# ariel415el/SoundEventDetection-Pytorch

Hardware: AMD Instinct MI355X
Metric: SED train clips/sec (60s,64-mel,9-layer CNN) (higher is better)
Workload: dtype bf16; 1 GPU; Cnn_AvgPooling main widths [32, 64, 128, 128], 60 s / 32 kHz / 64-mel clips (T=6001 frames, NFFT 1024, hop 320), batch 32/GPU, train step = waveform->log-mel->fwd->BCE->bwd->Adam-amsgrad; frontend_constants=bench, graph_replay=False, global_batch=32, frames=6001, parallelism=dp1, frontend_in_step=True, frontend_overlapped=False, frontend_overlap_mode=0, sync_bn=False, rccl_group=False, collectives_executed=False

## Files before the change

### soundeventdetection-pytorch_amd/csrc/sed_c1.hip

```cpp
#include "conv_common.h"

constexpr int C1_TR = 8;

template <typename T>
__global__ __launch_bounds__(256) void conv_c1_fwd_kernel(const float* __restrict__ x, const float* __restrict__ mean,
                                                          const float* __restrict__ stdv, const float* __restrict__ w,
                                                          T* __restrict__ z, float* __restrict__ partial, int B,
                                                          int H, int W, int Cout, int Coutp, int G, int PPB) {
    extern __shared__ __attribute__((aligned(16))) char smem[];
    float* wsm = reinterpret_cast<float*>(smem);
    float* xrow = wsm + 9 * Coutp;
    float* red = xrow + (C1_TR + 2) * (W + 2);
    const int tid = threadIdx.x;
    for (int i = tid; i < 9 * Coutp; i += blockDim.x) {
        const int tap = i / Coutp, c = i % Coutp;
        wsm[i] = c < Cout ? w[c * 9 + tap] : 0.f;
    }
    __syncthreads();
    const int cg = tid % G, pl = tid / G;
    float wr[9][8];
#pragma unroll
    for (int t = 0; t < 9; ++t)
#pragma unroll
        for (int e = 0; e < 8; ++e) wr[t][e] = wsm[t * Coutp + cg * 8 + e];
    float S[8], Q[8];
#pragma unroll
    for (int e = 0; e < 8; ++e) { S[e] = 0.f; Q[e] = 0.f; }
    const int WP2 = W + 2;
    const int bands = (H + C1_TR - 1) / C1_TR;
    for (int band = blockIdx.x; band < B * bands; band += gridDim.x) {
        const int b = band / bands, h0 = (band - b * bands) * C1_TR;
        __syncthreads();
        for (int i = tid; i < (C1_TR + 2) * WP2; i += blockDim.x) {
            const int rr = i / WP2, cc = i - rr * WP2;
            const int hy = h0 + rr - 1, wx = cc - 1;
            float v = 0.f;
            if (hy >= 0 && hy < H && wx >= 0 && wx < W) {
                v = x[((size_t)b * H + hy) * W + wx];
                if (mean) v = (v - mean[wx]) / stdv[wx];
            }
            xrow[i] = v;
        }
        __syncthreads();
        if (pl < PPB) {
            for (int wq = pl; wq < W; wq += PPB) {
                float x0[3], x1[3], x2[3];
#pragma unroll
                for (int j = 0; j < 3; ++j) { x0[j] = xrow[wq + j]; x1[j] = xrow[WP2 + wq + j]; }
#pragma unroll
                for (int r = 0; r < C1_TR; ++r) {
#pragma unroll
                    for (int j = 0; j < 3; ++j) x2[j] = xrow[(r + 2) * WP2 + wq + j];
                    if (h0 + r < H) {
                        float a[8];
#pragma unroll
                        for (int e = 0; e < 8; ++e) a[e] = 0.f;
#pragma unroll
                        for (int j = 0; j < 3; ++j) {
#pragma unroll
                            for (int e = 0; e < 8; ++e) a[e] = fmaf(x0[j], wr[j][e], a[e]);
                        }
#pragma unroll
                        for (int j = 0; j < 3; ++j) {
#pragma unroll
                            for (int e = 0; e < 8; ++e) a[e] = fmaf(x1[j], wr[3 + j][e], a[e]);
                        }
#pragma unroll
                        for (int j = 0; j < 3; ++j) {
#pragma unroll
                            for (int e = 0; e < 8; ++e) a[e] = fmaf(x2[j], wr[6 + j][e], a[e]);
                        }
#pragma unroll
                        for (int e = 0; e < 8; ++e) { S[e] += a[e]; Q[e] = fmaf(a[e], a[e], Q[e]); }
                        store8<T>(z + (((size_t)b * H + h0 + r) * W + wq) * Coutp + cg * 8, a);
                    }
#pragma unroll
                    for (int j = 0; j < 3; ++j) { x0[j] = x1[j]; x1[j] = x2[j]; }
                }
            }
        }
    }
    if (partial) {
        __syncthreads();
        if (pl < PPB) {
#pragma unroll
            for (int e = 0; e < 8; ++e) {
                red[(pl * 2 + 0) * Coutp + cg * 8 + e] = S[e];
                red[(pl * 2 + 1) * Coutp + cg * 8 + e] = Q[e];
            }
        }
        __syncthreads();
        for (int i = tid; i < 2 * Coutp; i += blockDim.x) {
            float t = 0.f;
            for (int q = 0; q < PPB; ++q) t += red[q * 2 * Coutp + i];
            partial[(size_t)blockIdx.x * 2 * Coutp + i] = t;
        }
    }
}

template <typename T, bool FUSED, int NPF>
__global__ __launch_bounds__(256) void conv_c1_wgrad_kernel(const float* __restrict__ x, const float* __restrict__ mean,
                                                            const float* __restrict__ stdv, const T* __restrict__ dz,
                                                            const T* __restrict__ zsrc, const float* __restrict__ ca,
                                                            const float* __restrict__ cb, const float* __restrict__ cc,
                                                            float* __restrict__ partial, int B, int H, int W,
                                                            int Coutp, int G, int PPB) {
    extern __shared__ __attribute__((aligned(16))) char smem[];
    float* xrow = reinterpret_cast<float*>(smem);
    float* red = xrow + (C1_TR + 2) * (W + 2);
    const int tid = threadIdx.x;
    const int cg = tid % G, pl = tid / G;
    const int WP2 = W + 2;
    float acc[9][8];
#pragma unroll
    for (int t = 0; t < 9; ++t)
#pragma unroll
        for (int e = 0; e < 8; ++e) acc[t][e] = 0.f;
    float a8[8], b8[8], c8[8];
    if (FUSED) {
#pragma unroll
        for (int e = 0; e < 8; ++e) { a8[e] = ca[cg * 8 + e]; b8[e] = cb[cg * 8 + e]; c8[e] = cc[cg * 8 + e]; }
    }
    const int bands = (H + C1_TR - 1) / C1_TR;
    const int nstage = (C1_TR + 2) * WP2;
    float pf[NPF];
    auto fetch = [&](int band) {
        const int b = band / bands, h0 = (band - b * bands) * C1_TR;
#pragma unroll
        for (int u = 0; u < NPF; ++u) {
            const int i = tid + u * 256;
            const int rr = i / WP2, cc2 = i - rr * WP2;
            const int hy = h0 + rr - 1, wx = cc2 - 1;
            float v = 0.f;
            if (i < nstage && band < B * bands && hy >= 0 && hy < H && wx >= 0 && wx < W) {
                v = x[((size_t)b * H + hy) * W + wx];
                if (mean) v = (v - mean[wx]) / stdv[wx];
            }
            pf[u] = v;
        }
    };
    fetch(blockIdx.x);
    for (int band = blockIdx.x; band < B * bands; band += gridDim.x) {
        const int b = band / bands, h0 = (band - b * bands) * C1_TR;
        (void)b;
        __syncthreads();
#pragma unroll
        for (int u = 0; u < NPF; ++u)
            if (tid + u * 256 < nstage) xrow[tid + u * 256] = pf[u];
        __syncthreads();
        fetch(band + gridDim.x);
        if (pl < PPB) {
            for (int wq = pl; wq < W; wq += PPB) {
                float x0[3], x1[3], x2[3];
#pragma unroll
                for (int j = 0; j < 3; ++j) { x0[j] = xrow[wq + j]; x1[j] = xrow[WP2 + wq + j]; }
                float d[C1_TR][8], zz[FUSED ? C1_TR : 1][8];
#pragma unroll
                for (int r = 0; r < C1_TR; ++r) {
                    const int h = (h0 + r < H) ? h0 + r : H - 1;
                    const size_t off = (((size_t)b * H + h) * W + wq) * Coutp + cg * 8;
                    load8<T>(dz + off, d[r]);
                    if (FUSED) load8<T>(zsrc + off, zz[FUSED ? r : 0]);
                }
#pragma unroll
                for (int r = 0; r < C1_TR; ++r) {
#pragma unroll
                    for (int j = 0; j < 3; ++j) x2[j] = xrow[(r + 2) * WP2 + wq + j];
                    if (h0 + r < H) {
                        if (FUSED) {
#pragma unroll
                            for (int e = 0; e < 8; ++e) d[r][e] = fmaf(a8[e], d[r][e], fmaf(b8[e], zz[FUSED ? r : 0][e], c8[e]));
                        }
#pragma unroll
                        for (int j = 0; j < 3; ++j) {
#pragma unroll
                            for (int e = 0; e < 8; ++e) {
                                acc[j][e] = fmaf(x0[j], d[r][e], acc[j][e]);
                                acc[3 + j][e] = fmaf(x1[j], d[r][e], acc[3 + j][e]);
                                acc[6 + j][e] = fmaf(x2[j], d[r][e], acc[6 + j][e]);
                            }
                        }
                    }
#pragma unroll
                    for (int j = 0; j < 3; ++j) { x0[j] = x1[j]; x1[j] = x2[j]; }
                }
            }
        }
    }
#pragma unroll
    for (int t = 0; t < 9; ++t) {
        __syncthreads();
        if (pl < PPB) {
#pragma unroll
            for (int e = 0; e < 8; ++e) red[pl * Coutp + cg * 8 + e] = acc[t][e];
        }
        __syncthreads();
        for (int i = tid; i < Coutp; i += blockDim.x) {
            float sacc = 0.f;
            for (int q = 0; q < PPB; ++q) sacc += red[q * Coutp + i];
            partial[((size_t)blockIdx.x * 9 + t) * Coutp + i] = sacc;
        }
    }
}

template <int SIT>
__global__ __launch_bounds__(256) void conv_c1_gram_kernel(const float* __restrict__ x, const float* __restrict__ mean,
                                                           const float* __restrict__ stdv, float* __restrict__ partial,
                                                           int B, int H, int W) {
    extern __shared__ __attribute__((aligned(16))) char smem[];
    float* xrow = reinterpret_cast<float*>(smem);
    float* red = xrow + (C1_TR + 2) * (W + 2);
    const int tid = threadIdx.x, lane = tid & 63, wave = tid >> 6;
    const int WP2 = W + 2;
    float acc[54];
#pragma unroll
    for (int i = 0; i < 54; ++i) acc[i] = 0.f;
    const int bands = (H + C1_TR - 1) / C1_TR;
    int srow[SIT], scol[SIT];
    float smu[SIT], sinv[SIT];
#pragma unroll
    for (int u = 0; u < SIT; ++u) {
        const int i = tid + u * 256;
        const int rr = i / WP2, cc2 = i - rr * WP2;
        const bool ok = i < (C1_TR + 2) * WP2 && cc2 >= 1 && cc2 <= W;
        srow[u] = i < (C1_TR + 2) * WP2 ? rr - 1 : (1 << 28);
        scol[u] = ok ? cc2 - 1 : -1;
        smu[u] = (ok && mean) ? mean[cc2 - 1] : 0.f;
        sinv[u] = (ok && mean) ? 1.0f / stdv[cc2 - 1] : 1.f;
    }
    const int npix = C1_TR * W;
    float nraw[SIT];
    unsigned nvalid = 0;
    auto fetch = [&](int band) {
        nvalid = 0;
        if (band >= B * bands) return;
        const int b = band / bands, h0 = (band - b * bands) * C1_TR;
#pragma unroll
        for (int u = 0; u < SIT; ++u) {
            const int hy = h0 + srow[u];
            const bool ok = hy >= 0 && hy < H && scol[u] >= 0;
            nraw[u] = ok ? x[((size_t)b * H + hy) * W + scol[u]] : 0.f;
            nvalid |= ok ? (1u << u) : 0u;
        }
    };
    fetch(blockIdx.x);
    for (int band = blockIdx.x; band < B * bands; band += gridDim.x) {
        const int b = band / bands, h0 = (band - b * bands) * C1_TR;
        (void)b;
        __syncthreads();
#pragma unroll
        for (int u = 0; u < SIT; ++u) {
            const int i = tid + u * 256;
            if (i >= (C1_TR + 2) * WP2) break;
            xrow[i] = ((nvalid >> u) & 1u) ? (nraw[u] - smu[u]) * sinv[u] : 0.f;
        }
        fetch(band + gridDim.x);
        __syncthreads();
        for (int pix = tid; pix < npix; pix += blockDim.x) {
            const int r = pix / W, wq = pix - r * W;
            if (h0 + r >= H) continue;
            float xp[9];
#pragma unroll
            for (int t = 0; t < 9; ++t) xp[t] = xrow[(r + t / 3) * WP2 + wq + t % 3];
#pragma unroll
            for (int j = 0; j < 9; ++j)
#pragma unroll
                for (int k = j; k < 9; ++k) {
                    constexpr int dummy = 0; (void)dummy;
                    const int o = j * 9 - j * (j - 1) / 2 + (k - j);
                    acc[o] = fmaf(xp[j], xp[k], acc[o]);
                }
#pragma unroll
            for (int k = 0; k < 9; ++k) acc[45 + k] += xp[k];
        }
    }
    __syncthreads();
#pragma unroll
    for (int i = 0; i < 54; ++i) {
        const float t = wave_sum(acc[i]);
        if (lane == 0) red[wave * 54 + i] = t;
    }
    __syncthreads();
    if (tid < 54) partial[(size_t)blockIdx.x * 54 + tid] = red[tid] + red[54 + tid] + red[108 + tid] + red[162 + tid];
}

__global__ __launch_bounds__(1024) void bn_train_finalize_c1_kernel(const float* __restrict__ gram, int nparts, double count,
                                                                    const float* __restrict__ w, const float* __restrict__ gamma,
                                                                    const float* __restrict__ beta, float* __restrict__ rmean,
                                                                    float* __restrict__ rvar, float momentum, float eps,
                                                                    float* __restrict__ scale, float* __restrict__ shift,
                                                                    float* __restrict__ mean_o, float* __restrict__ invstd_o, int C,
                                                                    int Cp, double* __restrict__ gsum_out = nullptr) {
    __shared__ double G[54];
    __shared__ double Gp[16][64];
    const int tid = threadIdx.x;
    {
        const int v = tid & 63, g = tid >> 6;
        double s = 0.0;
        if (v < 54) {
            int i = g;
            for (; i + 16 * 7 < nparts; i += 16 * 8) {
                float t[8];
#pragma unroll
                for (int u = 0; u < 8; ++u) t[u] = gram[(size_t)(i + 16 * u) * 54 + v];
#pragma unroll
                for (int u = 0; u < 8; ++u) s += (double)t[u];
            }
            for (; i < nparts; i += 16) s += (double)gram[(size_t)i * 54 + v];
        }
        Gp[g][v] = s;
    }
    __syncthreads();
    if (tid < 54) {
        double s = 0.0;
        for (int g = 0; g < 16; ++g) s += Gp[g][tid];
        G[tid] = s;
        if (gsum_out != nullptr) gsum_out[tid] = s;
    }
    __syncthreads();
    for (int c = tid; c < Cp; c += blockDim.x) {
        if (c >= C) { scale[c] = 0.f; shift[c] = 0.f; mean_o[c] = 0.f; invstd_o[c] = 0.f; continue; }
        double s1 = 0.0, s2 = 0.0;
        for (int j = 0; j < 9; ++j) {
            s1 += (double)w[c * 9 + j] * G[45 + j];
            for (int k2 = 0; k2 < 9; ++k2) {
                const int a = j < k2 ? j : k2, b2 = j < k2 ? k2 : j;
                s2 += (double)w[c * 9 + j] * (double)w[c * 9 + k2] * G[a * 9 - a * (a - 1) / 2 + (b2 - a)];
            }
        }
        const double mean = s1 / count;
        double var = s2 / count - mean * mean;
        if (var < 0.0) var = 0.0;
        const float invstd = (float)(1.0 / sqrt(var + (double)eps));
        const float sc = gamma[c] * invstd;
        scale[c] = sc;
        shift[c] = beta[c] - (float)mean * sc;
        mean_o[c] = (float)mean;
        invstd_o[c] = invstd;
        if (rmean) {
            const double unbiased = count > 1.0 ? var * (count / (count - 1.0)) : var;
            rmean[c] = (1.f - momentum) * rmean[c] + momentum * (float)mean;
            rvar[c] = (1.f - momentum) * rvar[c] + momentum * (float)unbiased;
        }
    }
}

__global__ __launch_bounds__(256) void bn_bwd_finalize_c1_kernel(const float* __restrict__ partial, int nparts, double count,
                                                                 const float* __restrict__ A, const float* __restrict__ w,
                                                                 const float* __restrict__ gamma, const float* __restrict__ mean,
                                                                 const float* __restrict__ invstd, float* __restrict__ dgamma,
                                                                 float* __restrict__ dbeta, float* __restrict__ ca,
                                                                 float* __restrict__ cb, float* __restrict__ cc, int C, int Cp) {
    __shared__ double sm[256];
    const int c = blockIdx.x, tid = threadIdx.x;
    double s = 0.0;
    for (int i = tid; i < nparts; i += 256) s += (double)partial[((size_t)i * 2 + 0) * Cp + c];
    sm[tid] = s;
    __syncthreads();
    for (int o = 128; o > 0; o >>= 1) {
        if (tid < o) sm[tid] += sm[tid + o];
        __syncthreads();
    }
    if (tid == 0) {
        if (c >= C) { ca[c] = 0.f; cb[c] = 0.f; cc[c] = 0.f; return; }
        const double sg = sm[0];
        double sgz = 0.0;
        for (int k2 = 0; k2 < 9; ++k2) sgz += (double)w[c * 9 + k2] * (double)A[k2 * Cp + c];
        const double g = gamma[c], is = invstd[c], mu = mean[c];
        const double q = is * (sgz - mu * sg);
        dbeta[c] = (float)sg;
        dgamma[c] = (float)q;
        const double mg = sg / count, mgx = q / count;
        ca[c] = (float)(g * is);
        cb[c] = (float)(-g * is * is * mgx);
        cc[c] = (float)(-g * is * (mg - mu * is * mgx));
    }
}

__global__ __launch_bounds__(1024) void conv_c1_wgrad_combine_kernel(const float* __restrict__ A, const float* __restrict__ gram,
                                                                    int nparts, const float* __restrict__ w,
                                                                    const float* __restrict__ ca, const float* __restrict__ cb,
                                                                    const float* __restrict__ cc, float* __restrict__ dw,
                                                                    int Cout, int Coutp, float* __restrict__ dw_torch = nullptr) {
    __shared__ double G[54];
    __shared__ double Gp[16][64];
    const int tid = threadIdx.x;
    {
        const int v = tid & 63, g = tid >> 6;
        double s = 0.0;
        if (v < 54) {
            int i = g;
            for (; i + 16 * 7 < nparts; i += 16 * 8) {
                float t[8];
#pragma unroll
                for (int u = 0; u < 8; ++u) t[u] = gram[(size_t)(i + 16 * u) * 54 + v];
#pragma unroll
                for (int u = 0; u < 8; ++u) s += (double)t[u];
            }
            for (; i < nparts; i += 16) s += (double)gram[(size_t)i * 54 + v];
        }
        Gp[g][v] = s;
    }
    __syncthreads();
    if (tid < 54) {
        double s = 0.0;
        for (int g = 0; g < 16; ++g) s += Gp[g][tid];
        G[tid] = s;
    }
    __syncthreads();
    for (int idx = tid; idx < 9 * Coutp; idx += blockDim.x) {
        const int k = idx / Coutp, c = idx - k * Coutp;
        float out = 0.f;
        if (c < Cout) {
            double wg = 0.0;
            for (int j = 0; j < 9; ++j) {
                const int a = j < k ? j : k, b2 = j < k ? k : j;
                wg += (double)w[c * 9 + j] * G[a * 9 - a * (a - 1) / 2 + (b2 - a)];
            }
            out = (float)((double)ca[c] * (double)A[idx] + (double)cb[c] * wg + (double)cc[c] * G[45 + k]);
        }
        dw[idx] = out;
        if (dw_torch != nullptr && c < Cout) dw_torch[c * 9 + k] = out;
    }
}

__global__ __launch_bounds__(1024) void c1_bwd_tail_kernel(const float* __restrict__ a_part, int a_nparts, const double* __restrict__ gsum,
                                                           double count, const float* __restrict__ w, const float* __restrict__ gamma,
                                                           const float* __restrict__ mean, const float* __restrict__ invstd,
                                                           float* __restrict__ dgamma, float* __restrict__ dbeta, float* __restrict__ ca,
                                                           float* __restrict__ cb, float* __restrict__ cc, float* __restrict__ a10_out,
                                                           float* __restrict__ dw, int Cout, float* __restrict__ dw_torch) {
    constexpr int Cp = 32, NV = 10 * Cp, NG = 3;
    __shared__ double As[NG][NV];
    __shared__ float a10[NV];
    __shared__ float coef[3][Cp];
    __shared__ double G[54];
    const int tid = threadIdx.x;
    if (tid < 54) G[tid] = gsum[tid];
    if (tid < NG * NV) {
        const int v = tid % NV, g = tid / NV;
        double s = 0.0;
        int i = g;
        for (; i + NG * 7 < a_nparts; i += NG * 8) {
            float t[8];
#pragma unroll
            for (int u = 0; u < 8; ++u) t[u] = a_part[(size_t)(i + NG * u) * NV + v];
#pragma unroll
            for (int u = 0; u < 8; ++u) s += (double)t[u];
        }
        for (; i < a_nparts; i += NG) s += (double)a_part[(size_t)i * NV + v];
        As[g][v] = s;
    }
    __syncthreads();
    if (tid < NV) {
        const float t = (float)(As[0][tid] + As[1][tid] + As[2][tid]);
        a10[tid] = t;
        a10_out[tid] = t;
    }
    __syncthreads();
    if (tid < Cp) {
        const int c = tid;
        float fa = 0.f, fb = 0.f, fc = 0.f;
        if (c < Cout) {
            const double sg = (double)a10[9 * Cp + c];
            double sgz = 0.0;
            for (int k2 = 0; k2 < 9; ++k2) sgz += (double)w[c * 9 + k2] * (double)a10[k2 * Cp + c];
            const double g = gamma[c], is = invstd[c], mu = mean[c];
            const double q = is * (sgz - mu * sg);
            dbeta[c] = (float)sg;
            dgamma[c] = (float)q;
            const double mg = sg / count, mgx = q / count;
            fa = (float)(g * is);
            fb = (float)(-g * is * is * mgx);
            fc = (float)(-g * is * (mg - mu * is * mgx));
        }
        ca[c] = fa; cb[c] = fb; cc[c] = fc;
        coef[0][c] = fa; coef[1][c] = fb; coef[2][c] = fc;
    }
    __syncthreads();
    for (int idx = tid; idx < 9 * Cp; idx += blockDim.x) {
        const int k = idx / Cp, c = idx - k * Cp;
        float out = 0.f;
        if (c < Cout) {
            double wg = 0.0;
            for (int j = 0; j < 9; ++j) {
                const int a = j < k ? j : k, b2 = j < k ? k : j;
                wg += (double)w[c * 9 + j] * G[a * 9 - a * (a - 1) / 2 + (b2 - a)];
            }
            out = (float)((double)coef[0][c] * (double)a10[idx] + (double)coef[1][c] * wg + (double)coef[2][c] * G[45 + k]);
        }
        dw[idx] = out;
        if (dw_torch != nullptr && c < Cout) dw_torch[c * 9 + k] = out;
    }
}


extern "C" int sed_conv_c1_nparts(int B, int H, int W) {
    (void)W;
    const long long rows = (long long)B * H;
    return (int)(rows < 768 ? rows : 768);
}

static void c1_geometry(int Coutp, int* G, int* PPB, int* threads) {
    *G = Coutp / 8;
    *PPB = 256 / *G;
    if (*PPB < 1) *PPB = 1;
    *threads = 256;
}

extern "C" int sed_conv3x3_c1_fwd(int dtype, const float* x, const float* mean, const float* stdv, const float* w,
                                  void* z, float* stats_partial, int B, int H, int W, int Cout, int Coutp,
                                  void* stream) {
    SED_REQUIRE(Coutp % 32 == 0 && Coutp <= 2048 && Cout <= Coutp, "Coutp must be a multiple of 32, <= 2048");
    SED_REQUIRE((mean == nullptr) == (stdv == nullptr), "mean/std must both be given or both NULL");
    int G, PPB, threads;
    c1_geometry(Coutp, &G, &PPB, &threads);
    const int grid = sed_conv_c1_nparts(B, H, W);
    const size_t lds = ((size_t)9 * Coutp + (C1_TR + 2) * (size_t)(W + 2) + (size_t)PPB * 2 * Coutp) * sizeof(float);
    hipStream_t st = (hipStream_t)stream;
    if (dtype == SED_BF16)
        conv_c1_fwd_kernel<bf16_t><<<grid, threads, lds, st>>>(x, mean, stdv, w, (bf16_t*)z, stats_partial, B, H, W, Cout, Coutp, G, PPB);
    else if (dtype == SED_F32)
        conv_c1_fwd_kernel<float><<<grid, threads, lds, st>>>(x, mean, stdv, w, (float*)z, stats_partial, B, H, W, Cout, Coutp, G, PPB);
    else
        SED_REQUIRE(false, "bad dtype");
    SED_LAUNCH_CHECK();
    return 0;
}

static int c1_wgrad_common(int dtype, const float* x, const float* mean, const float* stdv, const void* dz,
                           const void* zsrc, const float* ca, const float* cb, const float* cc, float* dw_partial, int B,
                           int H, int W, int Coutp, void* stream);

static int c1_npf(int W) {
    const int n = (C1_TR + 2) * (W + 2);
    return W < 1 ? 0 : n <= 4 * 256 ? 4 : n <= 11 * 256 ? 11 : 0;
}

extern "C" int sed_conv3x3_c1_wgrad(int dtype, const float* x, const float* mean, const float* stdv, const void* dz,
                                    float* dw_partial, int B, int H, int W, int Coutp, void* stream) {
    return c1_wgrad_common(dtype, x, mean, stdv, dz, nullptr, nullptr, nullptr, nullptr, dw_partial, B, H, W, Coutp, stream);
}

extern "C" int sed_conv3x3_c1_wgrad_fused(int dtype, const float* x, const float* mean, const float* stdv,
                                          const void* g, const void* zsrc, const float* ca, const float* cb,
                                          const float* cc, float* dw_partial, int B, int H, int W, int Coutp,
                                          void* stream) {
    SED_REQUIRE(g && zsrc && ca && cb && cc, "fused dz operands");
    return c1_wgrad_common(dtype, x, mean, stdv, g, zsrc, ca, cb, cc, dw_partial, B, H, W, Coutp, stream);
}

static int c1_wgrad_common(int dtype, const float* x, const float* mean, const float* stdv, const void* dz,
                           const void* zsrc, const float* ca, const float* cb, const float* cc, float* dw_partial, int B,
                           int H, int W, int Coutp, void* stream) {
    SED_REQUIRE(Coutp % 32 == 0 && Coutp <= 2048, "Coutp must be a multiple of 32, <= 2048");
    int G, PPB, threads;
    c1_geometry(Coutp, &G, &PPB, &threads);
    const int grid = sed_conv_c1_nparts(B, H, W);
    const size_t lds = ((C1_TR + 2) * (size_t)(W + 2) + (size_t)PPB * Coutp) * sizeof(float);
    hipStream_t st = (hipStream_t)stream;
    const int npf = c1_npf(W);
    SED_REQUIRE(npf > 0, "W must be in [1, SED_ANYW_MAX_W]");
#define SED_C1W(N_)                                                                                                                         \
    if (dtype == SED_BF16)                                                                                                                  \
        if (zsrc) conv_c1_wgrad_kernel<bf16_t, true, N_><<<grid, threads, lds, st>>>(x, mean, stdv, (const bf16_t*)dz, (const bf16_t*)zsrc, ca, cb, cc, dw_partial, B, H, W, Coutp, G, PPB); \
        else conv_c1_wgrad_kernel<bf16_t, false, N_><<<grid, threads, lds, st>>>(x, mean, stdv, (const bf16_t*)dz, nullptr, ca, cb, cc, dw_partial, B, H, W, Coutp, G, PPB); \
    else if (dtype == SED_F32)                                                                                                              \
        if (zsrc) conv_c1_wgrad_kernel<float, true, N_><<<grid, threads, lds, st>>>(x, mean, stdv, (const float*)dz, (const float*)zsrc, ca, cb, cc, dw_partial, B, H, W, Coutp, G, PPB); \
        else conv_c1_wgrad_kernel<float, false, N_><<<grid, threads, lds, st>>>(x, mean, stdv, (const float*)dz, nullptr, ca, cb, cc, dw_partial, B, H, W, Coutp, G, PPB); \
    else                                                                                                                                    \
        SED_REQUIRE(false, "bad dtype");
    if (npf == 4) { SED_C1W(4) } else { SED_C1W(11) }
#undef SED_C1W
    SED_LAUNCH_CHECK();
    return 0;
}

extern "C" int sed_conv_c1_gram_nparts(int B, int H, int W) {
    (void)W;
    const long long bands = (long long)B * ((H + C1_TR - 1) / C1_TR);
    return (int)(bands < 2048 ? (bands < 1 ? 1 : bands) : 2048);
}

extern "C" int sed_conv3x3_c1_gram(const float* x, const float* mean, const float* stdv, float* gram_partial, int B, int H,
                                   int W, void* stream) {
    SED_REQUIRE((mean == nullptr) == (stdv == nullptr), "mean/std must both be given or both NULL");
    const int npf = c1_npf(W);
    SED_REQUIRE(npf > 0, "W must be in [1, SED_ANYW_MAX_W] (one band of input lines is staged by 256 threads)");
    const int grid = sed_conv_c1_gram_nparts(B, H, W);
    const size_t lds = ((C1_TR + 2) * (size_t)(W + 2) + 4 * 54) * sizeof(float);
    if (npf == 4) conv_c1_gram_kernel<4><<<grid, 256, lds, (hipStream_t)stream>>>(x, mean, stdv, gram_partial, B, H, W);
    else conv_c1_gram_kernel<11><<<grid, 256, lds, (hipStream_t)stream>>>(x, mean, stdv, gram_partial, B, H, W);
    SED_LAUNCH_CHECK();
    return 0;
}

extern "C" int sed_conv3x3_c1_wgrad_combine(const float* a_sum, const float* gram_partial, int nparts, const float* w,
                                            const float* ca, const float* cb, const float* cc, float* dwpack, int Cout,
                                            int Coutp, void* stream) {
    SED_REQUIRE(a_sum && gram_partial && w && ca && cb && cc && dwpack && nparts > 0, "operands");
    conv_c1_wgrad_combine_kernel<<<1, 1024, 0, (hipStream_t)stream>>>(a_sum, gram_partial, nparts, w, ca, cb, cc, dwpack, Cout, Coutp);
    SED_LAUNCH_CHECK();
    return 0;
}

extern "C" int sed_conv3x3_c1_wgrad_combine_u(const float* a_sum, const float* gram_partial, int nparts, const float* w,
                                              const float* ca, const float* cb, const float* cc, float* dwpack, int Cout,
                                              int Coutp, float* dw, void* stream) {
    SED_REQUIRE(a_sum && gram_partial && w && ca && cb && cc && dwpack && dw && nparts > 0, "operands");
    conv_c1_wgrad_combine_kernel<<<1, 1024, 0, (hipStream_t)stream>>>(a_sum, gram_partial, nparts, w, ca, cb, cc, dwpack, Cout, Coutp, dw);
    SED_LAUNCH_CHECK();
    return 0;
}

extern "C" int sed_bn_train_finalize_c1(const float* gram_partial, int nparts, double count, const float* w1, const float* gamma,
                                        const float* beta, float* running_mean, float* running_var, float momentum, float eps,
                                        float* scale, float* shift, float* mean, float* invstd, int C, int Cp, void* stream) {
    SED_REQUIRE(nparts > 0 && count > 0 && C <= Cp, "bad sizes");
    SED_REQUIRE((running_mean == nullptr) == (running_var == nullptr), "running stats must both be given or both NULL");
    bn_train_finalize_c1_kernel<<<1, 1024, 0, (hipStream_t)stream>>>(gram_partial, nparts, count, w1, gamma, beta, running_mean,
                                                                     running_var, momentum, eps, scale, shift, mean, invstd, C, Cp);
    SED_LAUNCH_CHECK();
    return 0;
}

extern "C" int sed_bn_train_finalize_c1_g(const float* gram_partial, int nparts, double count, const float* w1, const float* gamma,
                                          const float* beta, float* running_mean, float* running_var, float momentum, float eps,
                                          float* scale, float* shift, float* mean, float* invstd, int C, int Cp, double* gram_sum,
                                          void* stream) {
    SED_REQUIRE(nparts > 0 && count > 0 && C <= Cp && gram_sum, "bad sizes / operands");
    SED_REQUIRE((running_mean == nullptr) == (running_var == nullptr), "running stats must both be given or both NULL");
    bn_train_finalize_c1_kernel<<<1, 1024, 0, (hipStream_t)stream>>>(gram_partial, nparts, count, w1, gamma, beta, running_mean,
                                                                     running_var, momentum, eps, scale, shift, mean, invstd, C, Cp, gram_sum);
    SED_LAUNCH_CHECK();
    return 0;
}

extern "C" int sed_c1_bwd_tail(const float* a_partial, int a_nparts, const double* gram_sum, double count, const float* w1,
                               const float* gamma, const float* mean, const float* invstd, float* dgamma, float* dbeta, float* ca,
                               float* cb, float* cc, float* a_sum, float* dwpack, int Cout, int Coutp, float* dw, void* stream) {
    SED_REQUIRE(a_partial && gram_sum && w1 && gamma && mean && invstd && dgamma && dbeta && ca && cb && cc && a_sum && dwpack &&
                a_nparts > 0 && count > 0, "operands");
    SED_REQUIRE(Coutp == 32 && Cout > 0 && Cout <= 32, "covered: 32 (padded) conv1 channels");
    c1_bwd_tail_kernel<<<1, 1024, 0, (hipStream_t)stream>>>(a_partial, a_nparts, gram_sum, count, w1, gamma, mean, invstd, dgamma, dbeta,
                                                            ca, cb, cc, a_sum, dwpack, Cout, dw);
    SED_LAUNCH_CHECK();
    return 0;
}

extern "C" int sed_c1_mode_supported(int dtype, int W, int C1, int Cout2) {
    return dtype == SED_BF16 && W == 64 && C1 == 32 && Cout2 == 32;
}

static int c1_conv_common(ConvParams& p, int W, void* stream) {
    p.dbg = sed_dbg_env();
    p.wres = 0;
    p.nparts = sed_conv_nparts(p.B, p.H, W);
    const int rc = launch_conv_pc(p, W, (hipStream_t)stream);
    if (rc < 0) { sed_set_error("C1 mode: shape not covered (needs bf16, W = 64, 32 conv1 channels)"); return 1; }
    if (rc) return rc;
    hipError_t e_ = hipGetLastError();
    if (e_ != hipSuccess) { sed_set_error(std::string("C1 mode launch failed: ") + hipGetErrorString(e_)); return 2; }
    return 0;
}

extern "C" int sed_conv3x3_fwd_c1(int dtype, int epi, const float* x1, const float* fmean, const float* fstd, const float* w1,
                                  const float* pro_scale, const float* pro_shift, const void* wpack, void* z, float* partial,
                                  void* relu_mask, int B, int H, int W, int Coutp, void* stream) {
    SED_REQUIRE(dtype == SED_BF16 && x1 && w1 && pro_scale && pro_shift && wpack && z, "operands");
    SED_REQUIRE((fmean == nullptr) == (fstd == nullptr), "mean/std must both be given or both NULL");
    SED_REQUIRE(epi == SED_EPI_STORE || (epi == SED_EPI_STATS && partial), "epilogue");
    ConvParams p = {};
    p.x = nullptr; p.pro_scale = pro_scale; p.pro_shift = pro_shift; p.wpack = wpack; p.z = z; p.partial = partial;
    p.B = B; p.H = H; p.Cinp = 32; p.Coutp = Coutp; p.pro = SED_PRO_C1; p.epi = epi;
    p.c1_x = x1; p.c1_mean = fmean; p.c1_std = fstd; p.c1_w = w1; p.c1_mask = relu_mask;
    return c1_conv_common(p, W, stream);
}

extern "C" int sed_conv3x3_dgrad_c1(int dtype, const void* dz, const void* wpack_t, void* g, const void* relu_mask, float* partial,
                                    int B, int H, int W, int Cinp, void* stream) {
    SED_REQUIRE(dtype == SED_BF16 && dz && wpack_t && g && relu_mask && partial, "operands");
    ConvParams p = {};
    p.x = dz; p.wpack = wpack_t; p.z = g; p.partial = partial;
    p.B = B; p.H = H; p.Cinp = Cinp; p.Coutp = 32; p.pro = SED_PRO_NONE; p.epi = SED_EPI_RELUBWD_C1;
    p.c1_mask = const_cast<void*>(relu_mask);
    return c1_conv_common(p, W, stream);
}

static int wgrad_fused_c1_impl(int dtype, const float* x1, const float* fmean, const float* fstd, const float* w1,
                               const float* pro_scale, const float* pro_shift, const void* gsrc, const void* zsrc,
                               const float* scale, const float* shift, const float* ca, const float* cb,
                               const float* cc, int pool, void* dz_out, float* dwpack, float* workspace, int B, int H,
                               int W, int Coutp, void* stream, float* dw, int Cout, int Cin) {
    SED_REQUIRE(dtype == SED_BF16 && x1 && w1 && pro_scale && pro_shift && gsrc && zsrc && scale && shift && ca && cb && cc &&
                dwpack, "operands");
    Wgrad2Params p = {};
    p.x = nullptr; p.pro_scale = pro_scale; p.pro_shift = pro_shift; p.dz = gsrc; p.zsrc = zsrc; p.scale = scale; p.shift = shift;
    p.ca = ca; p.cb = cb; p.cc = cc; p.dz_out = dz_out; p.ws = workspace;
    p.B = B; p.H = H; p.Cinp = 32; p.Coutp = Coutp; p.pro = SED_PRO_C1; p.pool = pool < 1 ? 1 : pool;
    p.c1_x = x1; p.c1_mean = fmean; p.c1_std = fstd; p.c1_w = w1;
    p.dbg = sed_dbg_env();
    const int rc = launch_wgrad3(DZ_POOL, p, W, (hipStream_t)stream);
    if (rc < 0) { sed_set_error("C1 mode weight gradient: shape not covered (needs W = 64, 32 -> 32 channels)"); return 1; }
    if (rc) return rc;
    hipError_t e_ = hipGetLastError();
    if (e_ != hipSuccess) { sed_set_error(std::string("C1 mode wgrad launch failed: ") + hipGetErrorString(e_)); return 2; }
    const size_t n = (size_t)9 * 32 * Coutp;
    reduce_wgrad_slabs(workspace, dwpack, p.strips, n, dw, Cout, Cin, 32, Coutp, (hipStream_t)stream);
    SED_LAUNCH_CHECK();
    return 0;
}

extern "C" int sed_conv3x3_wgrad_fused_c1(int dtype, const float* x1, const float* fmean, const float* fstd, const float* w1,
                                          const float* pro_scale, const float* pro_shift, const void* gsrc, const void* zsrc,
                                          const float* scale, const float* shift, const float* ca, const float* cb,
                                          const float* cc, int pool, void* dz_out, float* dwpack, float* workspace, int B, int H,
                                          int W, int Coutp, void* stream) {
    return wgrad_fused_c1_impl(dtype, x1, fmean, fstd, w1, pro_scale, pro_shift, gsrc, zsrc, scale, shift, ca, cb, cc, pool, dz_out,
                               dwpack, workspace, B, H, W, Coutp, stream, nullptr, 0, 0);
}

extern "C" int sed_conv3x3_wgrad_fused_c1_u(int dtype, const float* x1, const float* fmean, const float* fstd, const float* w1,
                                            const float* pro_scale, const float* pro_shift, const void* gsrc, const void* zsrc,
                                            const float* scale, const float* shift, const float* ca, const float* cb,
                                            const float* cc, int pool, void* dz_out, float* dwpack, float* workspace, int B, int H,
                                            int W, int Coutp, float* dw, int Cout, int Cin, void* stream) {
    SED_REQUIRE(dw && Cout > 0 && Cin > 0 && Cout <= Coutp && Cin <= 32, "unpacked gradient operands");
    return wgrad_fused_c1_impl(dtype, x1, fmean, fstd, w1, pro_scale, pro_shift, gsrc, zsrc, scale, shift, ca, cb, cc, pool, dz_out,
                               dwpack, workspace, B, H, W, Coutp, stream, dw, Cout, Cin);
}

extern "C" int sed_conv3x3_bwd_fused_c1_supported(int dtype, int W, int Coutp, int pool) {
    if (!(dtype == SED_BF16 && W == 64 && Coutp == 32 && pool == 2)) return 0;
    if (const char* e = sed_getenv("SED_BWD_FUSED_C1")) if (e[0] == '0') return 0;
    return 1;
}

extern "C" int sed_conv3x3_bwd_fused_c1(int dtype, const float* x1, const float* fmean, const float* fstd, const float* w1,
                                        const float* pro_scale, const float* pro_shift, const void* gsrc, const void* zsrc,
                                        const float* scale, const float* shift, const float* ca, const float* cb, const float* cc,
                                        int pool, const void* wpack_t, const void* relu_mask, float* a_partial, float* dwpack,
                                        float* workspace, int B, int H, int W, int Coutp, float* dw, int Cout, int Cin, void* stream) {
    SED_REQUIRE(sed_conv3x3_bwd_fused_c1_supported(dtype, W, Coutp, pool), "covered: bf16, W = 64, 32 -> 32 channels, 2x2 pooling");
    SED_REQUIRE(x1 && w1 && pro_scale && pro_shift && gsrc && zsrc && scale && shift && ca && cb && cc && wpack_t &&
                a_partial && dwpack && workspace && B > 0 && H > 0, "operands");
    SED_REQUIRE(relu_mask == nullptr, "the ReLU gate is derived from the rebuilt activation tile: relu_mask must be NULL");
    SED_REQUIRE((fmean == nullptr) == (fstd == nullptr), "mean/std must both be given or both NULL");
    SED_REQUIRE(dw == nullptr || (Cout > 0 && Cin > 0 && Cout <= 32 && Cin <= 32), "unpacked gradient operands");
    SED_REQUIRE((double)H * W * 32 * 2 < 2147483648.0, "one image must stay below 2 GiB");
    int nwg = 0;
    const int rc = launch_bwd_fused_c1(x1, fmean, fstd, w1, pro_scale, pro_shift, gsrc, zsrc, scale, shift, ca, cb, cc, wpack_t,
                                       a_partial, sed_conv_dgrad_c1_nparts(), workspace, B, H, &nwg, (hipStream_t)stream);
    SED_REQUIRE(rc >= 0, "not covered");
    if (rc) return rc;
    SED_LAUNCH_CHECK();
    const size_t n = (size_t)9 * 32 * 32;
    reduce_wgrad_slabs(workspace, dwpack, nwg, n, dw, Cout, Cin, 32, 32, (hipStream_t)stream);
    SED_LAUNCH_CHECK();
    return 0;
}

extern "C" int sed_bn_bwd_finalize_c1(const float* partial, int nparts, double count, const float* a_sum, const float* w1,
                                      const float* gamma, const float* mean, const float* invstd, float* dgamma, float* dbeta,
                                      float* ca, float* cb, float* cc, int C, int Cp, void* stream) {
    SED_REQUIRE(nparts > 0 && count > 0 && C <= Cp && a_sum && w1, "bad sizes");
    bn_bwd_finalize_c1_kernel<<<Cp, 256, 0, (hipStream_t)stream>>>(partial, nparts, count, a_sum, w1, gamma, mean, invstd, dgamma,
                                                                   dbeta, ca, cb, cc, C, Cp);
    SED_LAUNCH_CHECK();
    return 0;
}
```

Baseline: 7742 clips/s.

## Compute conv1 input Gram via row-pair correlations with edge corrections

Replaces the per-pixel 45-entry 9-tap outer-product accumulation in the first-layer Gram kernel with a Toeplitz-style scheme. Each thread accumulates 13 row-shift correlations plus a sum over contiguous runs loaded as float2 windows. The 54 Gram entries are then rebuilt from these sums, minus boundary-row, boundary-column and corner corrections that are accumulated separately. Staging is also rewritten to use contiguous source reads with a padded LDS row stride, and the SIT and RUN template arguments are chosen from W. This cuts FMA count and register pressure in the gram pass, at the cost of intricate index-mapping logic and different float summation order.

```diff
diff --git a/soundeventdetection-pytorch_amd/csrc/sed_c1.hip b/soundeventdetection-pytorch_amd/csrc/sed_c1.hip
--- a/soundeventdetection-pytorch_amd/csrc/sed_c1.hip
+++ b/soundeventdetection-pytorch_amd/csrc/sed_c1.hip
@@ -203,85 +203,186 @@
     }
 }
 
-template <int SIT>
+constexpr int C1_GQ = 38;
+
+template <int N>
+__device__ __forceinline__ void c1_gram_window(const float* __restrict__ p, float (&a)[N]) {
+    if constexpr (N % 2 == 0) {
+#pragma unroll
+        for (int i = 0; i < N; i += 2) {
+            const float2 t = *reinterpret_cast<const float2*>(p + i);
+            a[i] = t.x; a[i + 1] = t.y;
+        }
+    } else {
+#pragma unroll
+        for (int i = 0; i < N; ++i) a[i] = p[i];
+    }
+}
+
+template <int SIT, int RUN>
 __global__ __launch_bounds__(256) void conv_c1_gram_kernel(const float* __restrict__ x, const float* __restrict__ mean,
                                                            const float* __restrict__ stdv, float* __restrict__ partial,
                                                            int B, int H, int W) {
     extern __shared__ __attribute__((aligned(16))) char smem[];
+    const int WS = ((W + 1) & ~1) + 8;
     float* xrow = reinterpret_cast<float*>(smem);
-    float* red = xrow + (C1_TR + 2) * (W + 2);
+    float* red = xrow + (C1_TR + 2) * WS;
+    float* erow = red + 4 * C1_GQ;
     const int tid = threadIdx.x, lane = tid & 63, wave = tid >> 6;
-    const int WP2 = W + 2;
-    float acc[54];
-#pragma unroll
-    for (int i = 0; i < 54; ++i) acc[i] = 0.f;
+    for (int i = tid; i < ((C1_TR + 2) * WS + 4 * C1_GQ + 8 * 256) / 4; i += 256) reinterpret_cast<float4*>(xrow)[i] = make_float4(0.f, 0.f, 0.f, 0.f);
     const int bands = (H + C1_TR - 1) / C1_TR;
-    int srow[SIT], scol[SIT];
+    const int nstage = (C1_TR + 2) * W;
+    int sidx[SIT];
     float smu[SIT], sinv[SIT];
+    const int q256 = 256 / W, r256 = 256 - q256 * W;
+    int rr = tid / W, cc = tid - rr * W;
 #pragma unroll
     for (int u = 0; u < SIT; ++u) {
-        const int i = tid + u * 256;
-        const int rr = i / WP2, cc2 = i - rr * WP2;
-        const bool ok = i < (C1_TR + 2) * WP2 && cc2 >= 1 && cc2 <= W;
-        srow[u] = i < (C1_TR + 2) * WP2 ? rr - 1 : (1 << 28);
-        scol[u] = ok ? cc2 - 1 : -1;
-        smu[u] = (ok && mean) ? mean[cc2 - 1] : 0.f;
-        sinv[u] = (ok && mean) ? 1.0f / stdv[cc2 - 1] : 1.f;
-    }
-    const int npix = C1_TR * W;
+        const bool ok = tid + u * 256 < nstage;
+        sidx[u] = ok ? rr * WS + 4 + cc : (1 << 28);
+        smu[u] = (ok && mean) ? mean[cc] : 0.f;
+        sinv[u] = (ok && mean) ? 1.0f / stdv[cc] : 1.f;
+        rr += q256; cc += r256;
+        if (cc >= W) { cc -= W; ++rr; }
+    }
     float nraw[SIT];
     unsigned nvalid = 0;
+    int nh0 = 0;
     auto fetch = [&](int band) {
         nvalid = 0;
         if (band >= B * bands) return;
-        const int b = band / bands, h0 = (band - b * bands) * C1_TR;
+        const int b = band / bands;
+        nh0 = (band - b * bands) * C1_TR;
+        const float* src = x + ((size_t)b * H + nh0) * W;
+        const int lim = (H - nh0 < C1_TR + 2 ? H - nh0 : C1_TR + 2) * WS;
 #pragma unroll
         for (int u = 0; u < SIT; ++u) {
-            const int hy = h0 + srow[u];
-            const bool ok = hy >= 0 && hy < H && scol[u] >= 0;
-            nraw[u] = ok ? x[((size_t)b * H + hy) * W + scol[u]] : 0.f;
+            const bool ok = sidx[u] < lim;
+            nraw[u] = ok ? src[tid + u * 256] : 0.f;
             nvalid |= ok ? (1u << u) : 0u;
         }
     };
+    float R0[3], R1[5], R2[5], T = 0.f;
+    float E4[4];
+#pragma unroll
+    for (int i = 0; i < 5; ++i) { R1[i] = 0.f; R2[i] = 0.f; }
+#pragma unroll
+    for (int i = 0; i < 3; ++i) R0[i] = 0.f;
+#pragma unroll
+    for (int i = 0; i < 4; ++i) E4[i] = 0.f;
+    const int RPR = (W + RUN - 1) / RUN;
+    bool any_edge = false;
     fetch(blockIdx.x);
     for (int band = blockIdx.x; band < B * bands; band += gridDim.x) {
-        const int b = band / bands, h0 = (band - b * bands) * C1_TR;
-        (void)b;
+        const int h0 = nh0;
         __syncthreads();
 #pragma unroll
         for (int u = 0; u < SIT; ++u) {
-            const int i = tid + u * 256;
-            if (i >= (C1_TR + 2) * WP2) break;
-            xrow[i] = ((nvalid >> u) & 1u) ? (nraw[u] - smu[u]) * sinv[u] : 0.f;
+            if (tid + u * 256 >= nstage) break;
+            xrow[sidx[u]] = ((nvalid >> u) & 1u) ? (nraw[u] - smu[u]) * sinv[u] : 0.f;
         }
         fetch(band + gridDim.x);
         __syncthreads();
-        for (int pix = tid; pix < npix; pix += blockDim.x) {
-            const int r = pix / W, wq = pix - r * W;
-            if (h0 + r >= H) continue;
-            float xp[9];
-#pragma unroll
-            for (int t = 0; t < 9; ++t) xp[t] = xrow[(r + t / 3) * WP2 + wq + t % 3];
-#pragma unroll
-            for (int j = 0; j < 9; ++j)
-#pragma unroll
-                for (int k = j; k < 9; ++k) {
-                    constexpr int dummy = 0; (void)dummy;
-                    const int o = j * 9 - j * (j - 1) / 2 + (k - j);
-                    acc[o] = fmaf(xp[j], xp[k], acc[o]);
+        const bool edge_band = h0 == 0 || H - 1 - h0 < C1_TR;
+        for (int q = tid; q < C1_TR * RPR; q += 256) {
+            const int r = q & (C1_TR - 1), c = q / C1_TR;
+            const float* l0 = xrow + r * WS + 4 + c * RUN;
+            float a0[RUN + 2], a1[RUN + 4], a2[RUN + 4];
+            c1_gram_window(l0, a0);
+            c1_gram_window(l0 + WS - 2, a1);
+            c1_gram_window(l0 + 2 * WS - 2, a2);
+#pragma unroll
+            for (int p = 0; p < RUN; ++p) {
+                const float v = a0[p];
+#pragma unroll
+                for (int s = 0; s < 3; ++s) R0[s] = fmaf(v, a0[p + s], R0[s]);
+#pragma unroll
+                for (int s = 0; s < 5; ++s) { R1[s] = fmaf(v, a1[p + s], R1[s]); R2[s] = fmaf(v, a2[p + s], R2[s]); }
+                T += v;
+            }
+        }
+        if (edge_band) {
+            any_edge = true;
+            for (int q = tid; q < C1_TR * RPR; q += 256) {
+                const int r = q & (C1_TR - 1), c = q / C1_TR;
+                const bool rf = h0 + r == 0, rl = h0 + r == H - 1;
+                if (!(rf || rl)) continue;
+                float a0[RUN + 2], e[8];
+                c1_gram_window(xrow + r * WS + 4 + c * RUN, a0);
+#pragma unroll
+                for (int i = 0; i < 8; ++i) e[i] = erow[i * 256 + tid];
+#pragma unroll
+                for (int p = 0; p < RUN; ++p) {
+                    const float vf = rf ? a0[p] : 0.f, vl = rl ? a0[p] : 0.f;
+#pragma unroll
+                    for (int s = 0; s < 3; ++s) { e[s] = fmaf(vf, a0[p + s], e[s]); e[3 + s] = fmaf(vl, a0[p + s], e[3 + s]); }
+                    e[6] += vf; e[7] += vl;
                 }
 #pragma unroll
-            for (int k = 0; k < 9; ++k) acc[45 + k] += xp[k];
-        }
-    }
-    __syncthreads();
-#pragma unroll
-    for (int i = 0; i < 54; ++i) {
-        const float t = wave_sum(acc[i]);
-        if (lane == 0) red[wave * 54 + i] = t;
-    }
-    __syncthreads();
-    if (tid < 54) partial[(size_t)blockIdx.x * 54 + tid] = red[tid] + red[54 + tid] + red[108 + tid] + red[162 + tid];
+                for (int i = 0; i < 8; ++i) erow[i * 256 + tid] = e[i];
+            }
+        }
+        if (wave < 2 && lane < C1_TR) {
+            const float* pc = xrow + lane * WS + 4 + (wave ? W - 1 : 0);
+            const float v = pc[0];
+            E4[0] = fmaf(v, v, E4[0]); E4[1] = fmaf(v, pc[WS], E4[1]); E4[2] = fmaf(v, pc[2 * WS], E4[2]);
+            E4[3] += v;
+        }
+        if (edge_band && wave == 2 && lane < 4) {
+            const int rp = (lane & 2) ? H - 1 - h0 : -h0;
+            if (rp >= 0 && rp < C1_TR) {
+                const float v = xrow[rp * WS + 4 + ((lane & 1) ? W - 1 : 0)];
+                E4[0] = fmaf(v, v, E4[0]); E4[1] += v;
+            }
+        }
+    }
+    __syncthreads();
+    auto put = [&](int i, float v) {
+        const float t = wave_sum(v);
+        if (lane == 0) red[wave * C1_GQ + i] = t;
+    };
+#pragma unroll
+    for (int i = 0; i < 3; ++i) put(i, R0[i]);
+#pragma unroll
+    for (int i = 0; i < 5; ++i) { put(3 + i, R1[i]); put(8 + i, R2[i]); }
+    put(13, T);
+    if (any_edge) {
+#pragma unroll
+        for (int i = 0; i < 8; ++i) put(14 + i, erow[i * 256 + tid]);
+    }
+    if (wave < 2) {
+#pragma unroll
+        for (int i = 0; i < 3; ++i) put(22 + 3 * wave + i, E4[i]);
+        put(28 + wave, E4[3]);
+    } else if (wave == 2 && lane < 4) {
+        red[wave * C1_GQ + 30 + lane] = E4[0];
+        red[wave * C1_GQ + 34 + lane] = E4[1];
+    }
+    __syncthreads();
+    if (tid < 54) {
+        auto tot = [&](int i) { return red[i] + red[C1_GQ + i] + red[2 * C1_GQ + i] + red[3 * C1_GQ + i]; };
+        int ta, tb, qR, qE = -1, qC = -1, qK = -1;
+        if (tid < 45) {
+            int j = 0, o = tid;
+            while (o >= 9 - j) { o -= 9 - j; ++j; }
+            const int k = j + o, tc = k / 3, td = k - 3 * tc;
+            ta = j / 3; tb = j - 3 * ta;
+            const int r = tc - ta, s = td - tb;
+            qR = r == 0 ? s : (r == 1 ? 5 : 10) + s;
+            if (r == 0 && ta != 1) qE = (ta == 0 ? 17 : 14) + s;
+            if (s == 0 && tb != 1) qC = (tb == 0 ? 25 : 22) + r;
+            if (j == k && ta != 1 && tb != 1) qK = 30 + (ta == 0 ? 2 : 0) + (tb == 0 ? 1 : 0);
+        } else {
+            const int k = tid - 45;
+            ta = k / 3; tb = k - 3 * ta;
+            qR = 13;
+            if (ta != 1) qE = ta == 0 ? 21 : 20;
+            if (tb != 1) qC = tb == 0 ? 29 : 28;
+            if (ta != 1 && tb != 1) qK = 34 + (ta == 0 ? 2 : 0) + (tb == 0 ? 1 : 0);
+        }
+        const float vR = tot(qR), vE = qE >= 0 ? tot(qE) : 0.f, vC = qC >= 0 ? tot(qC) : 0.f, vK = qK >= 0 ? tot(qK) : 0.f;
+        partial[(size_t)blockIdx.x * 54 + tid] = (vR - vC) + (vK - vE);
+    }
 }
 
 __global__ __launch_bounds__(1024) void bn_train_finalize_c1_kernel(const float* __restrict__ gram, int nparts, double count,
@@ -582,15 +683,24 @@
     return (int)(bands < 2048 ? (bands < 1 ? 1 : bands) : 2048);
 }
 
+static int c1_gram_run(int W) {
+    const int one = (C1_TR * W + 255) / 256, two = 2 * ((C1_TR * ((W + 1) / 2) + 255) / 256);
+    return two <= one ? 2 : 1;
+}
+
 extern "C" int sed_conv3x3_c1_gram(const float* x, const float* mean, const float* stdv, float* gram_partial, int B, int H,
                                    int W, void* stream) {
     SED_REQUIRE((mean == nullptr) == (stdv == nullptr), "mean/std must both be given or both NULL");
     const int npf = c1_npf(W);
     SED_REQUIRE(npf > 0, "W must be in [1, SED_ANYW_MAX_W] (one band of input lines is staged by 256 threads)");
     const int grid = sed_conv_c1_gram_nparts(B, H, W);
-    const size_t lds = ((C1_TR + 2) * (size_t)(W + 2) + 4 * 54) * sizeof(float);
-    if (npf == 4) conv_c1_gram_kernel<4><<<grid, 256, lds, (hipStream_t)stream>>>(x, mean, stdv, gram_partial, B, H, W);
-    else conv_c1_gram_kernel<11><<<grid, 256, lds, (hipStream_t)stream>>>(x, mean, stdv, gram_partial, B, H, W);
+    const size_t lds = ((C1_TR + 2) * (size_t)(((W + 1) & ~1) + 8) + 4 * C1_GQ + 8 * 256) * sizeof(float);
+    const int sit = ((C1_TR + 2) * W + 255) / 256, run = c1_gram_run(W);
+#define SED_C1G(S_)                                                                                                                         \
+    if (run == 2) conv_c1_gram_kernel<S_, 2><<<grid, 256, lds, (hipStream_t)stream>>>(x, mean, stdv, gram_partial, B, H, W);                \
+    else conv_c1_gram_kernel<S_, 1><<<grid, 256, lds, (hipStream_t)stream>>>(x, mean, stdv, gram_partial, B, H, W);
+    if (sit <= 3) { SED_C1G(3) } else if (sit <= 4) { SED_C1G(4) } else { SED_C1G(11) }
+#undef SED_C1G
     SED_LAUNCH_CHECK();
     return 0;
 }
```

Result: no change. 7778 clips/s, median of 6 (+0.5%).
